# Amanda-Zheng/MR-GNAS

Measured on AMD Instinct MI355X. Metric: million edges/sec per supernet fwd+bwd step (FB15k-237, dim=200), higher is better.
Workload: dtype f32

## Files before the change

include/mrgnas.h:

```cpp
#ifndef MRGNAS_H
#define MRGNAS_H

#include <stdint.h>

#ifdef __cplusplus
extern "C" {
#endif

#define MRG_ABI_VERSION 23

#define MRG_OK            0
#define MRG_E_NULLPTR    -1
#define MRG_E_SHAPE      -2
#define MRG_E_ENUM       -3
#define MRG_E_WORKSPACE  -4

#define MRG_COMPOSE_MULT 0
#define MRG_COMPOSE_SUB  1
#define MRG_COMPOSE_ADD  2
#define MRG_REDUCE_SUM   0
#define MRG_REDUCE_MEAN  1
#define MRG_REDUCE_MAX   2
#define MRG_GCS_SUB      0
#define MRG_GCS_MUL      1
// ... 120 lines not shown
  const int32_t *valid_rows;
  const double *given[MRG_MIX_MAX_CANDIDATES];
  int32_t given_n[MRG_MIX_MAX_CANDIDATES];
  int64_t given_stride[MRG_MIX_MAX_CANDIDATES];
} mrg_gated_branch;
int mrg_mix_colstats(const float *const *y_host, int K, int64_t rows, int D, double *sums, void *ws,
                     const mrg_gated_branch *gated, void *stream);
int mrg_mix_finalize_fwd(const double *sums, const float *const *gamma_host, const float *const *beta_host,
                         float *const *rmean_host, float *const *rvar_host, int K, double total_rows, int D,
                         float eps, float momentum, float *coef, void *stream);
int mrg_mix_stats_coef(const float *const *y, const float *const *gamma, const float *const *beta,
                       float *const *running_mean, float *const *running_var, int K, int64_t rows, double total_rows,
                       int D, float eps, float momentum, float *coef, void *ws, const mrg_gated_branch *gated, void *stream);
int mrg_mix_fwd(const float *const *y_host, int K, const float *coef, const float *w, const float *addend, float *out,
                int64_t rows, int D, const mrg_gated_branch *gated, void *stream);
int mrg_mix_bwd_reduce(const float *g, const float *const *y_host, int K, const float *coef, const float *w,
                       float *red, void *ws, int64_t rows, int D, const mrg_gated_branch *gated, void *stream);
int mrg_mix_finalize_bwd(const float *red, int K, double total_rows, int D, float *coef2,
                         float *const *dgamma_host, float *const *dbeta_host, float *dw, const int32_t *valid_rows, void *stream);
int mrg_mix_bwd_apply(const float *g, const float *const *y_host, float *const *gy_host, int K,
                      const float *coef, const float *coef2, const float *w, const float *const *rs, const float *rs_scale,
                      const float *rs_self, const int64_t *rs_edge_rows, const int *rs_on, const float *const *rs_full,
                      const float *const *fold_s,
                      const float *const *fold_gate, float *const *fold_gs, const int *fold_add_from, int64_t rows, int D,
                      const mrg_gated_branch *gated, void *stream);

int64_t mrg_zero_workspace_bytes(int D);
int mrg_zero_colstats(const float *ent, const float *rel, const int32_t *ent_idx, const int32_t *rel_idx, const int *ops, int K,
                      int64_t rows, int D, double *sums, void *ws, void *stream);
int mrg_zero_stats_coef(const float *ent, const float *rel, const int32_t *ent_idx, const int32_t *rel_idx, const int *ops, int K,
// ... 261 lines not shown
```

mr-gnas_amd/_lib.py:

```python
import ctypes
import os
import re

import torch

_HERE = os.path.dirname(os.path.abspath(__file__))
LIB_PATH = os.environ.get("MRG_LIB_PATH") or os.path.join(_HERE, "lib", "libmrgnas_hip.so")
HEADER_PATH = os.path.join(os.path.dirname(_HERE), "include", "mrgnas.h")

ABI_VERSION = 23


class MrgnasLibraryError(RuntimeError):
    pass


class MrgnasError(RuntimeError):
    """A C-ABI call returned a non-zero code."""


_P, _I, _L, _F = ctypes.c_void_p, ctypes.c_int, ctypes.c_int64, ctypes.c_float

SIGNATURES = {
    "mrg_abi_version": (_I, []),
# ... 21 lines not shown
    "mrg_gate_row_colsum_blocks": (_L, [_L, _L, _L, _I, _I]),
    "mrg_gate_row_fwd_colsum": (_I, [_P, _P, _P, _P, _P, _P, _L, _L, _L, _I, _F, _P, _P, _L]),
    "mrg_gate_row_bwd": (_I, [_P, _P, _P, _P, _P, _P, _P, _P, _L, _L, _L, _I, _P]),
    "mrg_gate_row_bwd_acc": (_I, [_P, _P, _P, _P, _P, _P, _P, _P, _L, _L, _L, _I, _P, _P]),
    "mrg_mix_workspace_bytes": (_L, [_I, _I]),
    "mrg_mix_colstats": (_I, [_P, _I, _L, _I, _P, _P, _P, _P]),
    "mrg_mix_finalize_fwd": (_I, [_P, _P, _P, _P, _P, _I, ctypes.c_double, _I, _F, _F, _P, _P]),
    "mrg_mix_stats_coef": (_I, [_P, _P, _P, _P, _P, _I, _L, ctypes.c_double, _I, _F, _F, _P, _P, _P, _P]),
    "mrg_zero_workspace_bytes": (_L, [_I]),
    "mrg_zero_colstats": (_I, [_P, _P, _P, _P, _P, _I, _L, _I, _P, _P, _P]),
    "mrg_zero_stats_coef": (_I, [_P, _P, _P, _P, _P, _I, _P, _P, _P, _P, _L, ctypes.c_double, _I, _F, _F, _P, _P, _P, _P]),
    "mrg_zero_fwd": (_I, [_P, _P, _P, _P, _P, _I, _P, _P, _P, _L, _I, _P, _P]),
    "mrg_zero_bwd_reduce": (_I, [_P, _P, _P, _P, _P, _P, _I, _P, _P, _P, _P, _L, _I, _P, _P]),
    "mrg_zero_bwd_apply": (_I, [_P, _P, _P, _P, _P, _P, _I, _P, _P, _P, _P, _P, _L, _I, _P, _P]),
    "mrg_mix_fwd": (_I, [_P, _I, _P, _P, _P, _P, _L, _I, _P, _P]),
    "mrg_mix_bwd_reduce": (_I, [_P, _P, _I, _P, _P, _P, _P, _L, _I, _P, _P]),
    "mrg_mix_finalize_bwd": (_I, [_P, _I, ctypes.c_double, _I, _P, _P, _P, _P, _P, _P]),
    "mrg_mix_bwd_apply": (_I, [_P, _P, _P, _I, _P, _P, _P, _P, _P, _P, _P, _P, _P, _P, _P, _P, _P, _L, _I, _P, _P]),
    "mrg_dense_filter_fwd": (_I, [_I, _P, _P, _P, _P, _P, _F, _P, _P, _P, _L, _I, _P]),
    "mrg_dense_filter_dz": (_I, [_I, _P, _P, _P, _P, _F, _P, _P, _L, _I, _P]),
    "mrg_gemm_workspace_bytes": (_L, [_I, _I]),
    "mrg_gemm_set_mode": (_I, [_I]),
    "mrg_gemm_set_wide8": (_I, [_I]),
    "mrg_gemm_set_q": (_I, [_I]),
    "mrg_gemm_set_small": (_I, [_I]),
    "mrg_segmax_bwd_input_ok": (_I, [_I, _I]),
    "mrg_segmax_bwd_input": (_I, [_P, _P, _P, _P, _P, _P, _P, _P, _L, _L, _I, _I, _P]),
    "mrg_segmax_bwd_input_chain": (_I, [_P, _P, _P, _P, _P, _P, _P, _P, _L, _L, _I, _I, _P, _P, _P, _P]),
    "mrg_seg_std_workspace_bytes": (_L, [_L, _I]),
    "mrg_seg_std_fwd": (_I, [_P, _P, _P, _P, _P, _P, _L, _P, _P, _P, _L, _L, _P, _P, _P, _P, _P, _L, _I, _P]),
# ... 217 lines not shown
def ptr_array(tensors):
    arr = (ctypes.c_void_p * len(tensors))()
    for i, t in enumerate(tensors):
        arr[i] = None if t is None else t.data_ptr()
    return arr


class GatedBranch(ctypes.Structure):
    _fields_ = [("k", ctypes.c_int32), ("s", ctypes.c_void_p), ("rowscale", ctypes.c_void_p),
                ("row_k", ctypes.c_int32), ("row_f", ctypes.c_void_p), ("row_h", ctypes.c_void_p), ("row_uvc", ctypes.c_void_p),
                ("row_ld", ctypes.c_int32), ("b0", ctypes.c_int64), ("b1", ctypes.c_int64), ("row_dq", ctypes.c_void_p),
                ("act", ctypes.c_int32), ("valid_rows", ctypes.c_void_p),
                ("given", ctypes.c_void_p * 8), ("given_n", ctypes.c_int32 * 8), ("given_stride", ctypes.c_int64 * 8)]


class ColSums:

    __slots__ = ("buf", "offset", "n", "stride", "rows")

    def __init__(self, buf, offset, n, stride, rows):
        self.buf, self.offset, self.n, self.stride, self.rows = buf, int(offset), int(n), int(stride), int(rows)


ACTS = {"relu": 0, "tanh": 1}


def gated_branch(spec, row_dq=None, act=0, valid_rows=None, given=None):
    dp = lambda t: None if t is None else t.data_ptr()
    if given is not None and not any(c is not None for c in given):
        given = None
# ... 41 lines not shown
```

mr-gnas_amd/cell_lp.py:

```python
import os

import torch
import torch.nn as nn
import torch.nn.functional as F

from . import functional as K
from . import lazy as LZ
from . import operations_lp as OPS
from .operations_lp import PRE_OPS, FIRST_OPS, MIDDLE_OPS, LAST_OPS, MIXED_OPS, MIXED_OPS_sf, SF_OPS

CALLER = os.environ.get("MRG_CALLER", "fused")

MIXED_STREAMS = int(os.environ.get("MRG_MIXED_STREAMS", "1"))


def _literal(h):
    x = h.x if isinstance(h, K.Fan) else h
    return CALLER == "reference" or not (x.table if isinstance(x, K.LazyRows) else x).is_cuda


def _tensor(y):
    return y.y if isinstance(y, K.Candidate) else y


# ... 166 lines not shown
    def loss_1n(self, weights, all_ent, sub_emb, rel_emb, label_index, subj, rel, label_smooth=0.0, col_chunk=None):
        width = self._fused_width(weights, all_ent, sub_emb, rel_emb)
        gamma = self._ops[0][0].gamma if width else None
        if width == 2:
            return K.sf_mix_bce_all(all_ent, sub_emb, rel_emb, weights, gamma, label_index, subj, rel, label_smooth, col_chunk)
        if width == 3:
            hidden = self._ops[2][0].query(sub_emb, rel_emb)
            return K.sf_mix3_bce_all(all_ent, sub_emb, rel_emb, hidden, weights, gamma, label_index, subj, rel, label_smooth, col_chunk)
        return F.binary_cross_entropy(self.forward(weights, all_ent, sub_emb, rel_emb), label_index.labels(subj, rel, label_smooth))


def _dense_stage(mixed_ops, states, h_in, weights, g, steps, fan):
    off = 0
    for _ in range(steps):
        s = None
        for j, h in enumerate(states):
            s = mixed_ops[off + j](weights[off + j], g, h, h_in, addend=s)
        off += len(states)
        states.append(fan(s))
    return states


def _no_fan(x):
    return x


class Cell_Zero(nn.Module):
    def __init__(self, nodes, feature_dim, drop_aggr, registry=None):
        super().__init__()
        self._feature_dim = feature_dim
        self._ops = nn.ModuleList([MixedOp(feature_dim, drop_aggr, PRE_OPS, registry)])

# ... 87 lines not shown
```

mr-gnas_amd/csrc/mixedop.hip:

```cpp
#include "mixedop_parts.hpp"

namespace mrg {

struct RowScalePack { const float* rs[MRG_MIX_MAXK]; float scale[MRG_MIX_MAXK]; float self_scale[MRG_MIX_MAXK]; int64_t edge_rows[MRG_MIX_MAXK]; int on[MRG_MIX_MAXK];
                      const float* full[MRG_MIX_MAXK];
                      const float* s[MRG_MIX_MAXK]; const float* gate[MRG_MIX_MAXK]; float* gs_out[MRG_MIX_MAXK]; int add_from[MRG_MIX_MAXK]; };

struct GatedPack { int k; const float* s; const float* c;
                   int pair_k;
                   int rk; const float* rf;
                   const float* rh; const float* uvc; int uld; int64_t b0, b1; float* rdq;
                   const int32_t* vrows;
                   int act; };

__device__ __forceinline__ float gated_rowscale(const GatedPack& gp, int64_t r) { return gp.c[r]; }

template <int VEC, int LPR, int KMAX>
__device__ __forceinline__ void colstats_flush(const double (&s1)[KMAX][VEC], const double (&s2)[KMAX][VEC], double* red, double* __restrict__ dst,
                                               int D, int sl, int rw) {
  constexpr int RPB = MRG_BLOCK / LPR;
  constexpr int WIDTH = LPR * KMAX * VEC;
  __syncthreads();
#pragma unroll
  for (int q = 0; q < KMAX; ++q) {
// ... 195 lines not shown
  if (var < 0) var = 0;
  double invstd = 1.0 / sqrt(var + (double)eps);
  float g = gamma.p[k] ? gamma.p[k][c] : 1.f, b = beta.p[k] ? beta.p[k][c] : 0.f;
  float* o = coef + (int64_t)k * 4 * D;
  o[c] = (float)(g * invstd);
  o[D + c] = (float)(b - mean * g * invstd);
  o[2 * D + c] = (float)invstd;
  o[3 * D + c] = (float)(mean * invstd);
  if (rmean.p[k]) {
    double unbiased = total_rows > 1 ? var * (total_rows / (total_rows - 1.0)) : var;
    rmean.p[k][c] = (1.f - momentum) * rmean.p[k][c] + momentum * (float)mean;
    rvar.p[k][c] = (1.f - momentum) * rvar.p[k][c] + momentum * (float)unbiased;
  }
}

template <int VEC, int LPR, int KMAX, bool GATED, int KB, int ACT = 0>
__global__ __launch_bounds__(MRG_BLOCK) void mix_fwd_k(PtrPack ys, int K, const float* __restrict__ coef, const float* __restrict__ w,
                                                       float* __restrict__ out, int64_t rows, int D,
                                                       const float* __restrict__ addend, GatedPack gp) {
  extern __shared__ float lds[];
  constexpr int RPB = MRG_BLOCK / LPR;
  const int sl = threadIdx.x % LPR, rw = row_group_of_thread<LPR>();
  const int dv = D / VEC;
  for (int t = threadIdx.x; t < K * 2 * D; t += MRG_BLOCK) {
    int k = t / (2 * D), rem = t - k * 2 * D;
    lds[t] = coef[(int64_t)k * 4 * D + rem];
  }
  __syncthreads();
  float wk[KB];
#pragma unroll
  for (int k = 0; k < KB; ++k) wk[k] = k < K ? w[k] : 0.f;
  const int64_t nvalid = valid_rows(gp.vrows, rows);
  for (int64_t r = (int64_t)blockIdx.x * RPB + rw; r < rows; r += (int64_t)gridDim.x * RPB) {
    const bool pad = r >= nvalid;
#pragma unroll
    for (int q = 0; q < KMAX; ++q) {
      int c = sl + q * LPR;
      if (c < dv) {
        Vec<VEC> acc = addend ? Vec<VEC>::load(addend + r * D + c * VEC) : Vec<VEC>::fill(0.f);
        float gck = 1.f, rfv = 1.f;
        Vec<VEC> gsv = Vec<VEC>::fill(0.f);
        if constexpr (GATED) {
          gck = gated_rowscale(gp, r);
          rfv = gp.rf[r];
          gsv = Vec<VEC>::load(gp.s + r * D + c * VEC);
        }
        Vec<VEC> vin[KB];
#pragma unroll
        for (int k = 0; k < KB; ++k) {
          vin[k] = Vec<VEC>::fill(0.f);
          if (k < K && ys.p[k]) vin[k] = Vec<VEC>::load(ys.p[k] + r * D + c * VEC);
        }
#pragma unroll
        for (int k = 0; k < KB; ++k) {
          if (k < K) {
            Vec<VEC> v = vin[k];
            if constexpr (GATED) {
              const bool isg = k == gp.k;
              const float cm = isg ? gck : (k == gp.rk ? rfv : 1.0f);
#pragma unroll
              for (int j = 0; j < VEC; ++j) v[j] = v[j] * (isg ? gsv[j] : 1.0f) * cm;
            }
            Vec<VEC> sc = Vec<VEC>::load(lds + (k * 2 + 0) * D + c * VEC), sh = Vec<VEC>::load(lds + (k * 2 + 1) * D + c * VEC);
            if constexpr (ACT == 0) {
#pragma unroll
              for (int j = 0; j < VEC; ++j) {
                float z = v[j] * sc[j] + sh[j];
                acc[j] += wk[k] * (z > 0.f ? z : 0.f);
              }
            } else {
#pragma unroll
              for (int j = 0; j < VEC; ++j) acc[j] += wk[k] * tanhf(v[j] * sc[j] + sh[j]);
            }
          }
        }
        if (pad) acc = Vec<VEC>::fill(0.f);
        acc.store(out + r * D + c * VEC);
      }
    }
  }
}

template <int VEC, int LPR, int KMAX, int KB, bool GATED, int ACT = 0>
__global__ __launch_bounds__(MRG_BLOCK) void mix_bwd_reduce_k(const float* __restrict__ g, PtrPack ys, int K,
                                                              const float* __restrict__ coef, const float* __restrict__ w,
                                                              float* __restrict__ ws, int64_t rows, int D, GatedPack gp) {
  rows = valid_rows(gp.vrows, rows);
// ... 547 lines not shown

extern "C" int mrg_mix_finalize_fwd(const double* sums, const float* const* gamma_host, const float* const* beta_host,
                                    float* const* rmean_host, float* const* rvar_host, int K, double total_rows, int D,
                                    float eps, float momentum, float* coef, void* stream) {
  if (K < 1 || K > MRG_MIX_MAXK || D <= 0 || total_rows < 0) return MRG_E_SHAPE;
  if (!sums || !coef || !gamma_host || !beta_host) return MRG_E_NULLPTR;
  BnPacks bn;
  const int prc = bn_packs(&bn, gamma_host, beta_host, rmean_host, rvar_host, K);
  if (prc != MRG_OK) return prc;
  hipLaunchKernelGGL(mix_finalize_fwd_k, dim3((D + 127) / 128, K), dim3(128), 0, (hipStream_t)stream, sums, bn.gamma, bn.beta, bn.rmean, bn.rvar, K,
                     total_rows > 0 ? total_rows : 1.0, D, eps, momentum, coef, (const int32_t*)nullptr);
  MRG_LAUNCH_CHECK();
  return MRG_OK;
}

extern "C" int mrg_mix_fwd(const float* const* y_host, int K, const float* coef, const float* w, const float* addend, float* out,
                           int64_t rows, int D, const mrg_gated_branch* gated, void* stream) {
  if (!pack_ok((const void* const*)y_host, K) || rows < 0 || D <= 0) return MRG_E_SHAPE;
  if (rows == 0) return MRG_OK;
  if (!coef || !w || !out) return MRG_E_NULLPTR;
  hipStream_t st = (hipStream_t)stream;
  PtrPack ys{};
  bool al = aligned16(out) && aligned16(addend);
  for (int k = 0; k < K; ++k) { ys.p[k] = y_host[k]; al = al && aligned16(y_host[k]); }
  GatedPack gp;
  const int grc = gated_pack(gated, y_host, K, &gp, &al);
  if (grc != MRG_OK) return grc;
  RowGeom g = row_geom(D, al);
  if (!g.ok) return MRG_E_SHAPE;
  size_t lds = (size_t)K * 2 * D * sizeof(float);
  if (lds > 64 * 1024) return MRG_E_SHAPE;
#define CALL(V, L, KM)                                                                                    \
  do {                                                                                                    \
    const dim3 grid_(mix_fwd_grid(rows, L));                                                               \
    if (gp.act == 1) {                                                                                    \
      hipLaunchKernelGGL((mix_fwd_k<V, L, KM, false, 5, 1>), grid_, dim3(MRG_BLOCK), lds, st, ys, K, coef, w, out, rows, D, addend, gp); \
    } else if (gp.k >= 0 || gp.rk >= 0) {                                                                        \
      if (K <= 5) hipLaunchKernelGGL((mix_fwd_k<V, L, KM, true, 5>), grid_, dim3(MRG_BLOCK), lds, st, ys, K, coef, w, out, rows, D, addend, gp); \
      else hipLaunchKernelGGL((mix_fwd_k<V, L, KM, true, MRG_MIX_MAXK>), grid_, dim3(MRG_BLOCK), lds, st, ys, K, coef, w, out, rows, D, addend, gp); \
    } else {                                                                                              \
      if (K <= 5) hipLaunchKernelGGL((mix_fwd_k<V, L, KM, false, 5>), grid_, dim3(MRG_BLOCK), lds, st, ys, K, coef, w, out, rows, D, addend, gp); \
      else hipLaunchKernelGGL((mix_fwd_k<V, L, KM, false, MRG_MIX_MAXK>), grid_, dim3(MRG_BLOCK), lds, st, ys, K, coef, w, out, rows, D, addend, gp); \
    }                                                                                                     \
  } while (0)
  MRG_DISPATCH_GEOM(g, CALL);
#undef CALL
  MRG_LAUNCH_CHECK();
  return MRG_OK;
}

extern "C" int mrg_mix_bwd_reduce(const float* g, const float* const* y_host, int K, const float* coef, const float* w, float* red,
                                  void* ws, int64_t rows, int D, const mrg_gated_branch* gated, void* stream) {
  if (!pack_ok((const void* const*)y_host, K) || rows < 0 || D <= 0) return MRG_E_SHAPE;
  if (!coef || !w || !red || (rows > 0 && !g)) return MRG_E_NULLPTR;
  if (!ws) return MRG_E_WORKSPACE;
  hipStream_t st = (hipStream_t)stream;
  PtrPack ys{};
  bool al = aligned16(g);
  for (int k = 0; k < K; ++k) { ys.p[k] = y_host[k]; al = al && aligned16(y_host[k]); }
  GatedPack gp;
  const int grc = gated_pack(gated, y_host, K, &gp, &al);
  if (grc != MRG_OK) return grc;
  RowGeom gm = row_geom(D, al);
// ... 137 lines not shown
```

mr-gnas_amd/functional/__init__.py:

```python
from . import switches
from ._base import (
    bump_counters, deferred_counters,
    COMPOSE, REDUCE, ACT, gate_ld, same_rows, _same_memory, _cnt, _ws, _WS_BYTES, _ws_bytes, _chunk_plan_args, _SIDE_STREAMS,
    Fork,
)
from .candidates import (
    Link, Candidate, ForEpilogue, wants_stats,
)
from .gcs import (
    GCS, fused_gcs, span_gcs, ComposePlan, _ComposeAggregate, compose_aggregate,
)
from .reducers import (
    _seg_fwd, _heads_fwd, _seg_bwd, _SegReduce, seg_reduce, _AggRows, aggregate_rows, _fused_agg_ws, _LinReluAgg, linear_relu_aggregate,
    _LinReluPartial, linear_relu_partial, _SumPartial, sum_partial,
)
from .fanin import (
    sum_buffers, _Fanout, _FanBox, Fan,
)
from .compose_gather import (
    _Compose, compose, gather_rows, GatherPlan, _Gather, gather, LazyRows, _pair_meta, _GatherCompose,
)
from .gates import (
    _Gate, gate_comp, gate_last, _GateRow, gate_comp_row_factor,
)
from .row_linear import (
    _Linear, linear, module_linear,
)
from .dense import (
    _DenseFilter, _FoldHalves, dense_filter_comp, _DensePair, dense_pair_available, _GATED_C, _gated_rowscale, dense_filter_pair,
    dense_filter_single,
)
from .mixed import (
    _MixCfg, _ys_of, _MixedEpilogue, mixed_epilogue, PreparedEpilogue, _all_reduce_sum, StatChain,
    mixed_epilogue_prepare,
)
from .cell_zero import (
    _CellZeroMixed, cell_zero_mixed,
)
from .scoring import (
    ScorePlan, _DistMult, distmult_score, distmult_scores_all, _TransE, transe_scores_all,
    _BCE1N, rows_bce_all, dot_bce_all, distmult_bce_all, distmult_bce_mean, distmult_bce_dlogit, bce_default_col_chunk,
    transe_bce_all, transe_bce_mean, transe_bce_dlogit, cols_sum, score_bias_arg,
)
from .sf_mix import (
    _MixBCE1N, sf_mix_bce_all, sf_mix_bce_mean, sf_mix_bce_grad,
    _Mix3BCE1N, sf_mix3_bce_all, sf_mix3_bce_mean, sf_mix3_bce_grad,
)
from .ccorr import (
# ... 13 lines not shown
```

mr-gnas_amd/functional/mixed.py:

```python
import collections
import ctypes

import torch

from .. import _lib
from .._lib import ptr_array, call, f32c, ptr, require_hip, stream_of
from . import switches as SW
from ._base import _same_memory, _ws, _ws_bytes, bump_counters
from .candidates import Candidate
from .dense import _gated_rowscale


FoldedRowScale = collections.namedtuple("FoldedRowScale", "norm edge_rows scale_edge scale_self gated_link link slot")


class _MixCfg:

    def __init__(self, bns, present, group=None, total_rows=None, has_addend=False, rowscale=None, identity=None, gated=None, act=0,
                 valid_rows=None, given=None):
        self.bns, self.present, self.group, self.total_rows, self.has_addend = bns, present, group, total_rows, has_addend
        self.given = given
        self.act = act
        self.valid_rows = valid_rows
        self.gated = gated
# ... 2 lines not shown
        self.rowscale = rowscale


def _ys_of(cfg, stored):
    it = iter(stored)
    ys = [next(it) if p else None for p in cfg.present]
    if cfg.gated is not None and cfg.gated.get("row_k") is not None:
        ys[cfg.gated["row_k"]] = cfg.gated["s"]
    return ys


def _n_read(cfg, ys):
    return len({y.data_ptr() for y in ys if y is not None} | ({cfg.gated["s"].data_ptr()} if cfg.gated is not None else set()))


class _MixedEpilogue(torch.autograd.Function):
    @staticmethod
    def forward(ctx, cfg, w, *tensors):
        K_ = len(cfg.bns)
        nz = sum(cfg.present)
        ys_nz = [f32c(t) for t in tensors[:nz]]
        gam, bet = list(tensors[nz:nz + K_]), list(tensors[nz + K_:nz + 2 * K_])
        addend = f32c(tensors[nz + 2 * K_]) if cfg.has_addend else None
        ys = _ys_of(cfg, ys_nz)
        ref = next((y for y in ys if y is not None), None)
        if ref is None:
            raise _lib.MrgnasError("mixed epilogue needs at least one non-zero branch to know the row count")
        require_hip(w, addend, *ys_nz, *gam, *bet)
        rows, D = ref.shape
        dev, st = ref.device, stream_of(ref)
        w = f32c(w)
        total = float(cfg.total_rows if cfg.total_rows is not None else rows)
        coef = torch.empty(K_, 4, D, dtype=torch.float32, device=dev)
        ypa = ptr_array(ys)
        gb = _lib.gated_branch(cfg.gated, act=cfg.act, valid_rows=cfg.valid_rows)
        nz_rd = _n_read(cfg, ys)
        bn0 = cfg.bns[0]
        training = bn0.training or not bn0.track_running_stats
        if training:
            ws = _ws(_ws_bytes("mrg_mix_workspace_bytes", K_, D), ref)
            track = bn0.track_running_stats
            rm = ptr_array([b.running_mean if track else None for b in cfg.bns])
            rv = ptr_array([b.running_var if track else None for b in cfg.bns])
            mom = bn0.momentum if bn0.momentum is not None else 0.1
            if cfg.group is None:
                given, cfg.given = cfg.given, None
                if given is not None and cfg.valid_rows is None and all(c is None or c.rows == rows for c in given):
                    swept = set()
                    for k, y in enumerate(ys):
                        if y is not None and given[k] is None:
                            swept.add(y.data_ptr())
                            if cfg.gated is not None and k == cfg.gated.get("k"):
                                swept.add(cfg.gated["s"].data_ptr())
                    gb_stats = _lib.gated_branch(cfg.gated, act=cfg.act, given=given)
                    nb_stats = 4 * D * rows * len(swept) + sum(c.n * 2 * D * 8 for c in given if c is not None)
                else:
                    gb_stats, nb_stats = gb, 4 * D * rows * nz_rd
                call("mrg_mix_stats_coef", (ypa, ptr_array(gam), ptr_array(bet), rm, rv, K_, rows, total, D, bn0.eps, mom, ptr(coef), ptr(ws), gb_stats, st),
                     nbytes=nb_stats)
                del given
            else:
                if cfg.chain is not None and cfg.chain[0].sums is not None:
                    sums = cfg.chain[0].sums[cfg.chain[1]]
                else:
                    sums = torch.empty(K_, 2, D, dtype=torch.float64, device=dev)
                    call("mrg_mix_colstats", (ypa, K_, rows, D, ptr(sums), ptr(ws), gb, st), nbytes=4 * D * rows * nz_rd)
                    _all_reduce_sum(sums, cfg.group)
                call("mrg_mix_finalize_fwd", (ptr(sums), ptr_array(gam), ptr_array(bet), rm, rv, K_, total, D, bn0.eps, mom, ptr(coef), st))
            if track:
                bump_counters(cfg.bns)
        else:
            for k, b in enumerate(cfg.bns):
                invstd = torch.rsqrt(b.running_var + b.eps)
                coef[k, 0] = gam[k] * invstd
                coef[k, 1] = bet[k] - b.running_mean * gam[k] * invstd
                coef[k, 2] = invstd
                coef[k, 3] = b.running_mean * invstd
        out = torch.empty(rows, D, dtype=torch.float32, device=dev)
        call("mrg_mix_fwd", (ypa, K_, ptr(coef), ptr(w), ptr(addend), ptr(out), rows, D, gb, st), nbytes=4 * D * rows * (nz_rd + 1 + (addend is not None)))
        if SW.MASK_TAP is not None:
            masks = []
            for k in range(K_):
                one = torch.zeros(K_, dtype=torch.float32, device=dev)
                one[k] = 1.0
                o = torch.empty(rows, D, dtype=torch.float32, device=dev)
                call("mrg_mix_fwd", (ypa, K_, ptr(coef), ptr(one), None, ptr(o), rows, D, gb, st))
                masks.append(o > 0)
            SW.MASK_TAP(cfg.bns, masks)
        ctx.cfg, ctx.training, ctx.total, ctx.nz, ctx.nz_rd = cfg, training, total, nz, nz_rd
        ctx.save_for_backward(w, coef, *ys_nz)
        if cfg.chain is not None:
            cfg.chain[0].register(cfg.chain[1], ctx)
# ... 89 lines not shown
        else:
            on = rs_ptr = rs_edge = rs_scale = rs_self = rs_full = f_s = f_gate = f_gs_p = f_add = None
            n_fold = 0
        call("mrg_mix_bwd_apply", (ptr(g), ypa, ptr_array(gys), K_, ptr(coef), ptr(coef2), ptr(w), rs_ptr, rs_scale, rs_self, rs_edge, on, rs_full,
                                   f_s, f_gate, f_gs_p, f_add, rows, D, gb, st),
             nbytes=4 * D * rows * (1 + ctx.nz_rd + n_out + n_fold))
        if rs is not None:
            for k in range(K_):
                if rs[k] is not None and gys[k] is not None:
                    rs[k].link.written[rs[k].slot] = gys[k].data_ptr()
        dgam = [red_local[k, 1] for k in range(K_)]
        dbet = [red_local[k, 0] for k in range(K_)]
        return (None, dw, *gys_nz, *dgam, *dbet) + ((g,) if cfg.has_addend else ())


def mixed_epilogue(ys, bns, w, group=None, total_rows=None, addend=None, fold_row_scales=False, identity=None, act="relu",
                   valid_rows=None):
    return mixed_epilogue_prepare(ys, bns, group, total_rows, fold_row_scales, identity, act, valid_rows)(w, addend)


class PreparedEpilogue:

    def __init__(self, cfg, cand, bns):
        self.cfg, self.cand, self.bns = cfg, cand, bns

    def __call__(self, w, addend=None):
        self.cfg.has_addend = addend is not None
        tensors = self.cand + [b.weight for b in self.bns] + [b.bias for b in self.bns] + ([addend] if addend is not None else [])
        return _MixedEpilogue.apply(self.cfg, w, *tensors)

# ... 134 lines not shown
```

mr-gnas_amd/functional/switches.py:

```python
import os

ROW_FACTOR = os.environ.get("MRG_ROW_FACTOR", "1") == "1"
LAZY_ASUM = os.environ.get("MRG_LAZY_ASUM", "1") == "1"
FANIN_CHAIN = os.environ.get("MRG_FANIN_CHAIN", "1") == "1"
FUSED_AMAX = os.environ.get("MRG_FUSED_AMAX", "1") == "1"
FUSED_AMAX_MIN_ROWS = int(os.environ.get("MRG_FUSED_AMAX_MIN_ROWS", "100000"))
FUSED_AMEAN = os.environ.get("MRG_FUSED_AMEAN", "1") == "1"
WIDE_BWD_INPUT = os.environ.get("MRG_WIDE_BWD_INPUT", "1") == "1"
NODE_LINEAR = os.environ.get("MRG_NODE_LINEAR", "1") == "1"
MASK_TAP = None
FOLD_IDENTITY = os.environ.get("MRG_FOLD_IDENTITY", "1") == "1"
CELL_ZERO_FUSED = os.environ.get("MRG_CELL_ZERO_FUSED", "1") == "1"
FORK_MIN_ROWS = int(os.environ.get("MRG_FORK_MIN_ROWS", str(1 << 17)))
SEGMENT_STREAMS = int(os.environ.get("MRG_SEGMENT_STREAMS", "3"))
FOLD_ROW_SCALE = os.environ.get("MRG_FOLD_ROW_SCALE", "1") == "1"
GROUPED_SEGMENTS = os.environ.get("MRG_GROUPED_SEGMENTS", "1") == "1"
DENSE_PAIR = os.environ.get("MRG_DENSE_PAIR", "1") == "1"
GATED_RECOMPUTE = os.environ.get("MRG_GATED_RECOMPUTE", "1") == "1"
PRODUCER_STATS = os.environ.get("MRG_PRODUCER_STATS", "1") == "1"
COMPGCN_TAIL = os.environ.get("MRG_COMPGCN_TAIL", "1") == "1"
SPARSE_AMAX_BWD = os.environ.get("MRG_SPARSE_AMAX_BWD", "1") == "1"
CAND_LINEAR_GROUP = os.environ.get("MRG_CAND_LINEAR_GROUP", "1") == "1"
CCORR_PATH = None
```

Baseline: 11.72.

## Fuse per-state mixed-op epilogues of a cell step into one grouped forward kernel

Adds a grouped mixed-epilogue forward kernel that evaluates up to three mixed ops (one per input state) in a single launch and sums them directly. Before, each op's output was written and then re-read as the next op's addend. The intent is to remove the intermediate partial-sum round trips through memory and cut the number of launches per cell step. Backward reuses the per-member epilogue backward in sequence. The cost is more template instantiations, higher LDS use for the stacked coefficients, and stricter eligibility: no group, no valid_rows, ReLU only, K≤5, and matching shapes.

Result: no change. 11.76 (median of 6 runs) (+0.4%).

```diff
diff --git a/include/mrgnas.h b/include/mrgnas.h
--- a/include/mrgnas.h
+++ b/include/mrgnas.h
@@ -158,6 +158,16 @@
                        int D, float eps, float momentum, float *coef, void *ws, const mrg_gated_branch *gated, void *stream);
 int mrg_mix_fwd(const float *const *y_host, int K, const float *coef, const float *w, const float *addend, float *out,
                 int64_t rows, int D, const mrg_gated_branch *gated, void *stream);
+#define MRG_MIX_GROUP_MAX 3
+typedef struct mrg_mix_member {
+  const float *const *y;
+  int32_t K;
+  const float *coef;
+  const float *w;
+  const mrg_gated_branch *gated;
+} mrg_mix_member;
+int mrg_mix_fwd_group(const mrg_mix_member *members, int n_members, const float *addend, float *out, int64_t rows, int D,
+                      void *stream);
 int mrg_mix_bwd_reduce(const float *g, const float *const *y_host, int K, const float *coef, const float *w,
                        float *red, void *ws, int64_t rows, int D, const mrg_gated_branch *gated, void *stream);
 int mrg_mix_finalize_bwd(const float *red, int K, double total_rows, int D, float *coef2,
diff --git a/mr-gnas_amd/_lib.py b/mr-gnas_amd/_lib.py
--- a/mr-gnas_amd/_lib.py
+++ b/mr-gnas_amd/_lib.py
@@ -59,6 +59,7 @@
     "mrg_zero_bwd_reduce": (_I, [_P, _P, _P, _P, _P, _P, _I, _P, _P, _P, _P, _L, _I, _P, _P]),
     "mrg_zero_bwd_apply": (_I, [_P, _P, _P, _P, _P, _P, _I, _P, _P, _P, _P, _P, _L, _I, _P, _P]),
     "mrg_mix_fwd": (_I, [_P, _I, _P, _P, _P, _P, _L, _I, _P, _P]),
+    "mrg_mix_fwd_group": (_I, [_P, _I, _P, _P, _L, _I, _P]),
     "mrg_mix_bwd_reduce": (_I, [_P, _P, _I, _P, _P, _P, _P, _L, _I, _P, _P]),
     "mrg_mix_finalize_bwd": (_I, [_P, _I, ctypes.c_double, _I, _P, _P, _P, _P, _P, _P]),
     "mrg_mix_bwd_apply": (_I, [_P, _P, _P, _I, _P, _P, _P, _P, _P, _P, _P, _P, _P, _P, _P, _P, _P, _L, _I, _P, _P]),
@@ -306,6 +307,13 @@
                 ("given", ctypes.c_void_p * 8), ("given_n", ctypes.c_int32 * 8), ("given_stride", ctypes.c_int64 * 8)]
 
 
+MIX_GROUP_MAX = 3
+
+
+class MixMember(ctypes.Structure):
+    _fields_ = [("y", ctypes.c_void_p), ("K", ctypes.c_int32), ("coef", ctypes.c_void_p), ("w", ctypes.c_void_p), ("gated", ctypes.c_void_p)]
+
+
 class ColSums:
 
     __slots__ = ("buf", "offset", "n", "stride", "rows")
diff --git a/mr-gnas_amd/cell_lp.py b/mr-gnas_amd/cell_lp.py
--- a/mr-gnas_amd/cell_lp.py
+++ b/mr-gnas_amd/cell_lp.py
@@ -204,8 +204,12 @@
     off = 0
     for _ in range(steps):
         s = None
-        for j, h in enumerate(states):
-            s = mixed_ops[off + j](weights[off + j], g, h, h_in, addend=s)
+        if K.switches.GROUP_STATE_EPILOGUES and len(states) > 1 and not any(_literal(h) or isinstance(h, K.LazyRows) for h in states):
+            ws = [weights[off + j] for j in range(len(states))]
+            s = K.mixed_epilogue_group([mixed_ops[off + j](ws[j], g, h, h_in, prepare_only=True) for j, h in enumerate(states)], ws)
+        else:
+            for j, h in enumerate(states):
+                s = mixed_ops[off + j](weights[off + j], g, h, h_in, addend=s)
         off += len(states)
         states.append(fan(s))
     return states
diff --git a/mr-gnas_amd/csrc/mixedop.hip b/mr-gnas_amd/csrc/mixedop.hip
--- a/mr-gnas_amd/csrc/mixedop.hip
+++ b/mr-gnas_amd/csrc/mixedop.hip
@@ -233,23 +233,35 @@
   }
 }
 
-template <int VEC, int LPR, int KMAX, bool GATED, int KB, int ACT = 0>
-__global__ __launch_bounds__(MRG_BLOCK) void mix_fwd_k(PtrPack ys, int K, const float* __restrict__ coef, const float* __restrict__ w,
-                                                       float* __restrict__ out, int64_t rows, int D,
-                                                       const float* __restrict__ addend, GatedPack gp) {
+struct FwdMember { PtrPack ys; int K; const float* coef; const float* w; GatedPack gp; };
+template <int NM> struct FwdGroup { FwdMember m[NM]; };
+static_assert(sizeof(FwdGroup<MRG_MIX_GROUP_MAX>) <= 1024, "the members' packs are a small part of the 4 KB argument block");
+
+template <int VEC, int LPR, int KMAX, bool GATED, int KB, int ACT = 0, int NM = 1>
+__global__ __launch_bounds__(MRG_BLOCK) void mix_fwd_k(FwdGroup<NM> grp, float* __restrict__ out, int64_t rows, int D,
+                                                       const float* __restrict__ addend) {
   extern __shared__ float lds[];
   constexpr int RPB = MRG_BLOCK / LPR;
   const int sl = threadIdx.x % LPR, rw = row_group_of_thread<LPR>();
   const int dv = D / VEC;
-  for (int t = threadIdx.x; t < K * 2 * D; t += MRG_BLOCK) {
-    int k = t / (2 * D), rem = t - k * 2 * D;
-    lds[t] = coef[(int64_t)k * 4 * D + rem];
+  int lb[NM];
+  float wk[NM][KB];
+  int base = 0;
+#pragma unroll
+  for (int m = 0; m < NM; ++m) {
+    const int K = grp.m[m].K;
+    lb[m] = base;
+    base += K * 2 * D;
+    const float* __restrict__ coef = grp.m[m].coef;
+    for (int t = threadIdx.x; t < K * 2 * D; t += MRG_BLOCK) {
+      int k = t / (2 * D), rem = t - k * 2 * D;
+      lds[lb[m] + t] = coef[(int64_t)k * 4 * D + rem];
+    }
+#pragma unroll
+    for (int k = 0; k < KB; ++k) wk[m][k] = k < K ? grp.m[m].w[k] : 0.f;
   }
   __syncthreads();
-  float wk[KB];
-#pragma unroll
-  for (int k = 0; k < KB; ++k) wk[k] = k < K ? w[k] : 0.f;
-  const int64_t nvalid = valid_rows(gp.vrows, rows);
+  const int64_t nvalid = valid_rows(grp.m[0].gp.vrows, rows);
   for (int64_t r = (int64_t)blockIdx.x * RPB + rw; r < rows; r += (int64_t)gridDim.x * RPB) {
     const bool pad = r >= nvalid;
 #pragma unroll
@@ -257,39 +269,46 @@
       int c = sl + q * LPR;
       if (c < dv) {
         Vec<VEC> acc = addend ? Vec<VEC>::load(addend + r * D + c * VEC) : Vec<VEC>::fill(0.f);
-        float gck = 1.f, rfv = 1.f;
-        Vec<VEC> gsv = Vec<VEC>::fill(0.f);
-        if constexpr (GATED) {
-          gck = gated_rowscale(gp, r);
-          rfv = gp.rf[r];
-          gsv = Vec<VEC>::load(gp.s + r * D + c * VEC);
-        }
-        Vec<VEC> vin[KB];
-#pragma unroll
-        for (int k = 0; k < KB; ++k) {
-          vin[k] = Vec<VEC>::fill(0.f);
-          if (k < K && ys.p[k]) vin[k] = Vec<VEC>::load(ys.p[k] + r * D + c * VEC);
-        }
-#pragma unroll
-        for (int k = 0; k < KB; ++k) {
-          if (k < K) {
-            Vec<VEC> v = vin[k];
-            if constexpr (GATED) {
-              const bool isg = k == gp.k;
-              const float cm = isg ? gck : (k == gp.rk ? rfv : 1.0f);
-#pragma unroll
-              for (int j = 0; j < VEC; ++j) v[j] = v[j] * (isg ? gsv[j] : 1.0f) * cm;
-            }
-            Vec<VEC> sc = Vec<VEC>::load(lds + (k * 2 + 0) * D + c * VEC), sh = Vec<VEC>::load(lds + (k * 2 + 1) * D + c * VEC);
-            if constexpr (ACT == 0) {
-#pragma unroll
-              for (int j = 0; j < VEC; ++j) {
-                float z = v[j] * sc[j] + sh[j];
-                acc[j] += wk[k] * (z > 0.f ? z : 0.f);
+#pragma unroll
+        for (int m = 0; m < NM; ++m) {
+          const GatedPack& gp = grp.m[m].gp;
+          const PtrPack& ys = grp.m[m].ys;
+          const int K = grp.m[m].K;
+          const float* cl = lds + lb[m];
+          float gck = 1.f, rfv = 1.f;
+          Vec<VEC> gsv = Vec<VEC>::fill(0.f);
+          if constexpr (GATED) {
+            gck = gated_rowscale(gp, r);
+            rfv = gp.rf[r];
+            gsv = Vec<VEC>::load(gp.s + r * D + c * VEC);
+          }
+          Vec<VEC> vin[KB];
+#pragma unroll
+          for (int k = 0; k < KB; ++k) {
+            vin[k] = Vec<VEC>::fill(0.f);
+            if (k < K && ys.p[k]) vin[k] = Vec<VEC>::load(ys.p[k] + r * D + c * VEC);
+          }
+#pragma unroll
+          for (int k = 0; k < KB; ++k) {
+            if (k < K) {
+              Vec<VEC> v = vin[k];
+              if constexpr (GATED) {
+                const bool isg = k == gp.k;
+                const float cm = isg ? gck : (k == gp.rk ? rfv : 1.0f);
+#pragma unroll
+                for (int j = 0; j < VEC; ++j) v[j] = v[j] * (isg ? gsv[j] : 1.0f) * cm;
               }
-            } else {
-#pragma unroll
-              for (int j = 0; j < VEC; ++j) acc[j] += wk[k] * tanhf(v[j] * sc[j] + sh[j]);
+              Vec<VEC> sc = Vec<VEC>::load(cl + (k * 2 + 0) * D + c * VEC), sh = Vec<VEC>::load(cl + (k * 2 + 1) * D + c * VEC);
+              if constexpr (ACT == 0) {
+#pragma unroll
+                for (int j = 0; j < VEC; ++j) {
+                  float z = v[j] * sc[j] + sh[j];
+                  acc[j] += wk[m][k] * (z > 0.f ? z : 0.f);
+                }
+              } else {
+#pragma unroll
+                for (int j = 0; j < VEC; ++j) acc[j] += wk[m][k] * tanhf(v[j] * sc[j] + sh[j]);
+              }
             }
           }
         }
@@ -867,39 +886,68 @@
   return MRG_OK;
 }
 
+static int mix_fwd_members(const mrg_mix_member* mem, int nm, const float* addend, float* out, int64_t rows, int D, hipStream_t st) {
+  if (!mem || nm < 1 || nm > MRG_MIX_GROUP_MAX || rows < 0 || D <= 0) return MRG_E_SHAPE;
+  for (int m = 0; m < nm; ++m)
+    if (!pack_ok((const void* const*)mem[m].y, mem[m].K)) return MRG_E_SHAPE;
+  if (rows == 0) return MRG_OK;
+  if (!out) return MRG_E_NULLPTR;
+  FwdGroup<MRG_MIX_GROUP_MAX> grp{};
+  bool al = aligned16(out) && aligned16(addend);
+  bool gated = false;
+  size_t lds = 0;
+  int kmax = 0;
+  for (int m = 0; m < nm; ++m) {
+    FwdMember& fm = grp.m[m];
+    const int K = mem[m].K;
+    if (!mem[m].coef || !mem[m].w) return MRG_E_NULLPTR;
+    for (int k = 0; k < K; ++k) { fm.ys.p[k] = mem[m].y[k]; al = al && aligned16(mem[m].y[k]); }
+    fm.K = K; fm.coef = mem[m].coef; fm.w = mem[m].w;
+    const int grc = gated_pack(mem[m].gated, mem[m].y, K, &fm.gp, &al);
+    if (grc != MRG_OK) return grc;
+    const bool gm = fm.gp.k >= 0 || fm.gp.rk >= 0;
+    if (m > 0 && (gm != gated || fm.gp.vrows != grp.m[0].gp.vrows)) return MRG_E_SHAPE;
+    if (nm > 1 && (fm.gp.act != 0 || K > 5)) return MRG_E_SHAPE;
+    gated = gm;
+    lds += (size_t)K * 2 * D * sizeof(float);
+    if (K > kmax) kmax = K;
+  }
+  RowGeom g = row_geom(D, al);
+  if (!g.ok) return MRG_E_SHAPE;
+  if (lds > 64 * 1024) return MRG_E_SHAPE;
+  const int act = grp.m[0].gp.act;
+#define FWD(V, L, KM, GA, KB, ACT, NM)                                                                     \
+  do {                                                                                                    \
+    FwdGroup<NM> g_{};                                                                                     \
+    for (int m = 0; m < NM; ++m) g_.m[m] = grp.m[m];                                                        \
+    hipLaunchKernelGGL((mix_fwd_k<V, L, KM, GA, KB, ACT, NM>), grid_, dim3(MRG_BLOCK), lds, st, g_, out, rows, D, addend); \
+  } while (0)
+#define CALL(V, L, KM)                                                                                    \
+  do {                                                                                                    \
+    const dim3 grid_(mix_fwd_grid(rows, L));                                                               \
+    if (nm == 3) { if (gated) FWD(V, L, KM, true, 5, 0, 3); else FWD(V, L, KM, false, 5, 0, 3); }           \
+    else if (nm == 2) { if (gated) FWD(V, L, KM, true, 5, 0, 2); else FWD(V, L, KM, false, 5, 0, 2); }      \
+    else if (act == 1) FWD(V, L, KM, false, 5, 1, 1);                                                      \
+    else if (gated) { if (kmax <= 5) FWD(V, L, KM, true, 5, 0, 1); else FWD(V, L, KM, true, MRG_MIX_MAXK, 0, 1); }   \
+    else { if (kmax <= 5) FWD(V, L, KM, false, 5, 0, 1); else FWD(V, L, KM, false, MRG_MIX_MAXK, 0, 1); }  \
+  } while (0)
+  MRG_DISPATCH_GEOM(g, CALL);
+#undef CALL
+#undef FWD
+  MRG_LAUNCH_CHECK();
+  return MRG_OK;
+}
+
 extern "C" int mrg_mix_fwd(const float* const* y_host, int K, const float* coef, const float* w, const float* addend, float* out,
                            int64_t rows, int D, const mrg_gated_branch* gated, void* stream) {
   if (!pack_ok((const void* const*)y_host, K) || rows < 0 || D <= 0) return MRG_E_SHAPE;
-  if (rows == 0) return MRG_OK;
-  if (!coef || !w || !out) return MRG_E_NULLPTR;
-  hipStream_t st = (hipStream_t)stream;
-  PtrPack ys{};
-  bool al = aligned16(out) && aligned16(addend);
-  for (int k = 0; k < K; ++k) { ys.p[k] = y_host[k]; al = al && aligned16(y_host[k]); }
-  GatedPack gp;
-  const int grc = gated_pack(gated, y_host, K, &gp, &al);
-  if (grc != MRG_OK) return grc;
-  RowGeom g = row_geom(D, al);
-  if (!g.ok) return MRG_E_SHAPE;
-  size_t lds = (size_t)K * 2 * D * sizeof(float);
-  if (lds > 64 * 1024) return MRG_E_SHAPE;
-#define CALL(V, L, KM)                                                                                    \
-  do {                                                                                                    \
-    const dim3 grid_(mix_fwd_grid(rows, L));                                                               \
-    if (gp.act == 1) {                                                                                    \
-      hipLaunchKernelGGL((mix_fwd_k<V, L, KM, false, 5, 1>), grid_, dim3(MRG_BLOCK), lds, st, ys, K, coef, w, out, rows, D, addend, gp); \
-    } else if (gp.k >= 0 || gp.rk >= 0) {                                                                        \
-      if (K <= 5) hipLaunchKernelGGL((mix_fwd_k<V, L, KM, true, 5>), grid_, dim3(MRG_BLOCK), lds, st, ys, K, coef, w, out, rows, D, addend, gp); \
-      else hipLaunchKernelGGL((mix_fwd_k<V, L, KM, true, MRG_MIX_MAXK>), grid_, dim3(MRG_BLOCK), lds, st, ys, K, coef, w, out, rows, D, addend, gp); \
-    } else {                                                                                              \
-      if (K <= 5) hipLaunchKernelGGL((mix_fwd_k<V, L, KM, false, 5>), grid_, dim3(MRG_BLOCK), lds, st, ys, K, coef, w, out, rows, D, addend, gp); \
-      else hipLaunchKernelGGL((mix_fwd_k<V, L, KM, false, MRG_MIX_MAXK>), grid_, dim3(MRG_BLOCK), lds, st, ys, K, coef, w, out, rows, D, addend, gp); \
-    }                                                                                                     \
-  } while (0)
-  MRG_DISPATCH_GEOM(g, CALL);
-#undef CALL
-  MRG_LAUNCH_CHECK();
-  return MRG_OK;
+  const mrg_mix_member one{y_host, K, coef, w, gated};
+  return mix_fwd_members(&one, 1, addend, out, rows, D, (hipStream_t)stream);
+}
+
+extern "C" int mrg_mix_fwd_group(const mrg_mix_member* members, int n_members, const float* addend, float* out, int64_t rows, int D,
+                                 void* stream) {
+  return mix_fwd_members(members, n_members, addend, out, rows, D, (hipStream_t)stream);
 }
 
 extern "C" int mrg_mix_bwd_reduce(const float* g, const float* const* y_host, int K, const float* coef, const float* w, float* red,
diff --git a/mr-gnas_amd/functional/__init__.py b/mr-gnas_amd/functional/__init__.py
--- a/mr-gnas_amd/functional/__init__.py
+++ b/mr-gnas_amd/functional/__init__.py
@@ -31,7 +31,7 @@
     dense_filter_single,
 )
 from .mixed import (
-    _MixCfg, _ys_of, _MixedEpilogue, mixed_epilogue, PreparedEpilogue, _all_reduce_sum, StatChain,
+    _MixCfg, _ys_of, _MixedEpilogue, _MixedGroup, mixed_epilogue, mixed_epilogue_group, PreparedEpilogue, _all_reduce_sum, StatChain,
     mixed_epilogue_prepare,
 )
 from .cell_zero import (
diff --git a/mr-gnas_amd/functional/mixed.py b/mr-gnas_amd/functional/mixed.py
--- a/mr-gnas_amd/functional/mixed.py
+++ b/mr-gnas_amd/functional/mixed.py
@@ -40,68 +40,84 @@
     return len({y.data_ptr() for y in ys if y is not None} | ({cfg.gated["s"].data_ptr()} if cfg.gated is not None else set()))
 
 
+class _Member:
+
+    __slots__ = ("cfg", "training", "total", "nz", "nz_rd", "saved_tensors", "needs_input_grad", "ys", "gb", "rows", "D", "addend")
+
+
+def _coefficients(cfg, w, tensors):
+    K_ = len(cfg.bns)
+    nz = sum(cfg.present)
+    ys_nz = [f32c(t) for t in tensors[:nz]]
+    gam, bet = list(tensors[nz:nz + K_]), list(tensors[nz + K_:nz + 2 * K_])
+    addend = f32c(tensors[nz + 2 * K_]) if cfg.has_addend else None
+    ys = _ys_of(cfg, ys_nz)
+    ref = next((y for y in ys if y is not None), None)
+    if ref is None:
+        raise _lib.MrgnasError("mixed epilogue needs at least one non-zero branch to know the row count")
+    require_hip(w, addend, *ys_nz, *gam, *bet)
+    rows, D = ref.shape
+    dev, st = ref.device, stream_of(ref)
+    w = f32c(w)
+    total = float(cfg.total_rows if cfg.total_rows is not None else rows)
+    coef = torch.empty(K_, 4, D, dtype=torch.float32, device=dev)
+    ypa = ptr_array(ys)
+    gb = _lib.gated_branch(cfg.gated, act=cfg.act, valid_rows=cfg.valid_rows)
+    nz_rd = _n_read(cfg, ys)
+    bn0 = cfg.bns[0]
+    training = bn0.training or not bn0.track_running_stats
+    if training:
+        ws = _ws(_ws_bytes("mrg_mix_workspace_bytes", K_, D), ref)
+        track = bn0.track_running_stats
+        rm = ptr_array([b.running_mean if track else None for b in cfg.bns])
+        rv = ptr_array([b.running_var if track else None for b in cfg.bns])
+        mom = bn0.momentum if bn0.momentum is not None else 0.1
+        if cfg.group is None:
+            given, cfg.given = cfg.given, None
+            if given is not None and cfg.valid_rows is None and all(c is None or c.rows == rows for c in given):
+                swept = set()
+                for k, y in enumerate(ys):
+                    if y is not None and given[k] is None:
+                        swept.add(y.data_ptr())
+                        if cfg.gated is not None and k == cfg.gated.get("k"):
+                            swept.add(cfg.gated["s"].data_ptr())
+                gb_stats = _lib.gated_branch(cfg.gated, act=cfg.act, given=given)
+                nb_stats = 4 * D * rows * len(swept) + sum(c.n * 2 * D * 8 for c in given if c is not None)
+            else:
+                gb_stats, nb_stats = gb, 4 * D * rows * nz_rd
+            call("mrg_mix_stats_coef", (ypa, ptr_array(gam), ptr_array(bet), rm, rv, K_, rows, total, D, bn0.eps, mom, ptr(coef), ptr(ws), gb_stats, st),
+                 nbytes=nb_stats)
+            del given
+        else:
+            if cfg.chain is not None and cfg.chain[0].sums is not None:
+                sums = cfg.chain[0].sums[cfg.chain[1]]
+            else:
+                sums = torch.empty(K_, 2, D, dtype=torch.float64, device=dev)
+                call("mrg_mix_colstats", (ypa, K_, rows, D, ptr(sums), ptr(ws), gb, st), nbytes=4 * D * rows * nz_rd)
+                _all_reduce_sum(sums, cfg.group)
+            call("mrg_mix_finalize_fwd", (ptr(sums), ptr_array(gam), ptr_array(bet), rm, rv, K_, total, D, bn0.eps, mom, ptr(coef), st))
+        if track:
+            bump_counters(cfg.bns)
+    else:
+        for k, b in enumerate(cfg.bns):
+            invstd = torch.rsqrt(b.running_var + b.eps)
+            coef[k, 0] = gam[k] * invstd
+            coef[k, 1] = bet[k] - b.running_mean * gam[k] * invstd
+            coef[k, 2] = invstd
+            coef[k, 3] = b.running_mean * invstd
+    m = _Member()
+    m.cfg, m.training, m.total, m.nz, m.nz_rd, m.saved_tensors = cfg, training, total, nz, nz_rd, (w, coef, *ys_nz)
+    m.ys, m.gb, m.rows, m.D, m.addend = ys, gb, rows, D, addend
+    return m
+
+
 class _MixedEpilogue(torch.autograd.Function):
     @staticmethod
     def forward(ctx, cfg, w, *tensors):
-        K_ = len(cfg.bns)
-        nz = sum(cfg.present)
-        ys_nz = [f32c(t) for t in tensors[:nz]]
-        gam, bet = list(tensors[nz:nz + K_]), list(tensors[nz + K_:nz + 2 * K_])
-        addend = f32c(tensors[nz + 2 * K_]) if cfg.has_addend else None
-        ys = _ys_of(cfg, ys_nz)
-        ref = next((y for y in ys if y is not None), None)
-        if ref is None:
-            raise _lib.MrgnasError("mixed epilogue needs at least one non-zero branch to know the row count")
-        require_hip(w, addend, *ys_nz, *gam, *bet)
-        rows, D = ref.shape
-        dev, st = ref.device, stream_of(ref)
-        w = f32c(w)
-        total = float(cfg.total_rows if cfg.total_rows is not None else rows)
-        coef = torch.empty(K_, 4, D, dtype=torch.float32, device=dev)
-        ypa = ptr_array(ys)
-        gb = _lib.gated_branch(cfg.gated, act=cfg.act, valid_rows=cfg.valid_rows)
-        nz_rd = _n_read(cfg, ys)
-        bn0 = cfg.bns[0]
-        training = bn0.training or not bn0.track_running_stats
-        if training:
-            ws = _ws(_ws_bytes("mrg_mix_workspace_bytes", K_, D), ref)
-            track = bn0.track_running_stats
-            rm = ptr_array([b.running_mean if track else None for b in cfg.bns])
-            rv = ptr_array([b.running_var if track else None for b in cfg.bns])
-            mom = bn0.momentum if bn0.momentum is not None else 0.1
-            if cfg.group is None:
-                given, cfg.given = cfg.given, None
-                if given is not None and cfg.valid_rows is None and all(c is None or c.rows == rows for c in given):
-                    swept = set()
-                    for k, y in enumerate(ys):
-                        if y is not None and given[k] is None:
-                            swept.add(y.data_ptr())
-                            if cfg.gated is not None and k == cfg.gated.get("k"):
-                                swept.add(cfg.gated["s"].data_ptr())
-                    gb_stats = _lib.gated_branch(cfg.gated, act=cfg.act, given=given)
-                    nb_stats = 4 * D * rows * len(swept) + sum(c.n * 2 * D * 8 for c in given if c is not None)
-                else:
-                    gb_stats, nb_stats = gb, 4 * D * rows * nz_rd
-                call("mrg_mix_stats_coef", (ypa, ptr_array(gam), ptr_array(bet), rm, rv, K_, rows, total, D, bn0.eps, mom, ptr(coef), ptr(ws), gb_stats, st),
-                     nbytes=nb_stats)
-                del given
-            else:
-                if cfg.chain is not None and cfg.chain[0].sums is not None:
-                    sums = cfg.chain[0].sums[cfg.chain[1]]
-                else:
-                    sums = torch.empty(K_, 2, D, dtype=torch.float64, device=dev)
-                    call("mrg_mix_colstats", (ypa, K_, rows, D, ptr(sums), ptr(ws), gb, st), nbytes=4 * D * rows * nz_rd)
-                    _all_reduce_sum(sums, cfg.group)
-                call("mrg_mix_finalize_fwd", (ptr(sums), ptr_array(gam), ptr_array(bet), rm, rv, K_, total, D, bn0.eps, mom, ptr(coef), st))
-            if track:
-                bump_counters(cfg.bns)
-        else:
-            for k, b in enumerate(cfg.bns):
-                invstd = torch.rsqrt(b.running_var + b.eps)
-                coef[k, 0] = gam[k] * invstd
-                coef[k, 1] = bet[k] - b.running_mean * gam[k] * invstd
-                coef[k, 2] = invstd
-                coef[k, 3] = b.running_mean * invstd
+        m = _coefficients(cfg, w, tensors)
+        K_, (w, coef, *ys_nz) = len(cfg.bns), m.saved_tensors
+        ys, gb, rows, D, addend, training, total, nz, nz_rd = m.ys, m.gb, m.rows, m.D, m.addend, m.training, m.total, m.nz, m.nz_rd
+        dev, st, ypa = coef.device, stream_of(coef), ptr_array(ys)
         out = torch.empty(rows, D, dtype=torch.float32, device=dev)
         call("mrg_mix_fwd", (ypa, K_, ptr(coef), ptr(w), ptr(addend), ptr(out), rows, D, gb, st), nbytes=4 * D * rows * (nz_rd + 1 + (addend is not None)))
         if SW.MASK_TAP is not None:
@@ -221,6 +237,87 @@
         return (None, dw, *gys_nz, *dgam, *dbet) + ((g,) if cfg.has_addend else ())
 
 
+class _MixedGroup(torch.autograd.Function):
+
+    @staticmethod
+    def forward(ctx, cfgs, addend, *flat):
+        members, off = [], 0
+        for cfg in cfgs:
+            n = 1 + sum(cfg.present) + 2 * len(cfg.bns)
+            members.append(_coefficients(cfg, flat[off], flat[off + 1:off + n]))
+            off += n
+        addend = f32c(addend)
+        require_hip(addend)
+        m0 = members[0]
+        rows, D = m0.rows, m0.D
+        dev, st = m0.saved_tensors[1].device, stream_of(m0.saved_tensors[1])
+        out = torch.empty(rows, D, dtype=torch.float32, device=dev)
+        arr = (_lib.MixMember * len(members))()
+        keep, read = [], set()
+        for a, m in zip(arr, members):
+            ypa = ptr_array(m.ys)
+            keep.append(ypa)
+            a.y, a.K = ctypes.cast(ypa, ctypes.c_void_p), len(m.cfg.bns)
+            a.coef, a.w = m.saved_tensors[1].data_ptr(), m.saved_tensors[0].data_ptr()
+            a.gated = ctypes.addressof(m.gb._obj) if m.gb is not None else None
+            read |= {y.data_ptr() for y in m.ys if y is not None} | ({m.cfg.gated["s"].data_ptr()} if m.cfg.gated is not None else set())
+        call("mrg_mix_fwd", (arr, len(members), ptr(addend), ptr(out), rows, D, st), nbytes=4 * D * rows * (len(read) + 1 + (addend is not None)),
+             symbol="mrg_mix_fwd_group")
+        del keep
+        ctx.n_saved = [len(m.saved_tensors) for m in members]
+        ctx.save_for_backward(*[t for m in members for t in m.saved_tensors])
+        for m in members:
+            m.saved_tensors = m.ys = m.gb = m.addend = None
+        ctx.members, ctx.has_addend = members, addend is not None
+        return out
+
+    @staticmethod
+    def backward(ctx, g):
+        g = f32c(g)
+        saved, needs = ctx.saved_tensors, ctx.needs_input_grad
+        spans, off, pos = [], 0, 2
+        for m, n_s in zip(ctx.members, ctx.n_saved):
+            n_in = 1 + m.nz + 2 * len(m.cfg.bns)
+            spans.append((off, n_s, pos, n_in))
+            off, pos = off + n_s, pos + n_in
+        grads = [None] * len(ctx.members)
+        for j in reversed(range(len(ctx.members))):
+            m, (off, n_s, pos, n_in) = ctx.members[j], spans[j]
+            m.saved_tensors, m.needs_input_grad = saved[off:off + n_s], (False,) + tuple(needs[pos:pos + n_in])
+            grads[j] = _MixedEpilogue.backward(m, g)[1:1 + n_in]
+            m.saved_tensors = None
+        return (None, g if ctx.has_addend else None) + tuple(t for gr in grads for t in gr)
+
+
+def _groupable(preps):
+    if not SW.GROUP_STATE_EPILOGUES or SW.MASK_TAP is not None or not 2 <= len(preps) <= _lib.MIX_GROUP_MAX:
+        return False
+    shapes, gated = set(), set()
+    for p in preps:
+        c = p.cfg
+        if c.group is not None or c.valid_rows is not None or c.act != 0 or len(c.bns) > 5:
+            return False
+        ref = next((y for y in _ys_of(c, p.cand) if y is not None), None)
+        if ref is None or not ref.is_cuda:
+            return False
+        shapes.add((tuple(ref.shape), ref.device))
+        gated.add(c.gated is not None)
+    return len(shapes) == 1 and len(gated) == 1
+
+
+def mixed_epilogue_group(preps, ws, addend=None):
+    if len(preps) == 1 or not _groupable(preps):
+        s = addend
+        for p, w in zip(preps, ws):
+            s = p(w, s)
+        return s
+    flat = []
+    for p, w in zip(preps, ws):
+        p.cfg.has_addend = False
+        flat += [w] + p.cand + [b.weight for b in p.bns] + [b.bias for b in p.bns]
+    return _MixedGroup.apply([p.cfg for p in preps], addend, *flat)
+
+
 def mixed_epilogue(ys, bns, w, group=None, total_rows=None, addend=None, fold_row_scales=False, identity=None, act="relu",
                    valid_rows=None):
     return mixed_epilogue_prepare(ys, bns, group, total_rows, fold_row_scales, identity, act, valid_rows)(w, addend)
diff --git a/mr-gnas_amd/functional/switches.py b/mr-gnas_amd/functional/switches.py
--- a/mr-gnas_amd/functional/switches.py
+++ b/mr-gnas_amd/functional/switches.py
@@ -18,6 +18,7 @@
 DENSE_PAIR = os.environ.get("MRG_DENSE_PAIR", "1") == "1"
 GATED_RECOMPUTE = os.environ.get("MRG_GATED_RECOMPUTE", "1") == "1"
 PRODUCER_STATS = os.environ.get("MRG_PRODUCER_STATS", "1") == "1"
+GROUP_STATE_EPILOGUES = os.environ.get("MRG_GROUP_STATE_EPILOGUES", "1") == "1"
 COMPGCN_TAIL = os.environ.get("MRG_COMPGCN_TAIL", "1") == "1"
 SPARSE_AMAX_BWD = os.environ.get("MRG_SPARSE_AMAX_BWD", "1") == "1"
 CAND_LINEAR_GROUP = os.environ.get("MRG_CAND_LINEAR_GROUP", "1") == "1"
```
